# hank-kuo-cs/Volumetric-Primitives-Net

Hardware: AMD Instinct MI355X
Metric: render+Chamfer fwd+bwd images/sec (higher is better)
Workload: dtype f32; 1 GPU; C3: B=64/GPU (global 64), K=32 sphere primitives, 256x256 silhouette+depth, n=256 pts/prim (N=8192) vs M=2048 GT points, Chamfer+L1 fwd+bwd; global_batch=64, parallelism=dp1, collective=none, sampling=fresh Philox draws every step (device step counter, 28 steps drawn)

## Files before the change

### volumetric-primitives-net_amd/csrc/chamfer.hip

```cpp
#include "vpn_common.h"
#include "vpn_chamfer_feat.h"
#include "vpn_chamfer_loss.h"
#include "vpn_raster_common.h"
#include <stdlib.h>
#include <string.h>
#include <type_traits>

#pragma clang fp contract(off)

namespace vpn {

constexpr int CH_BLOCK = 256;
constexpr int CH_WTILE = 256;

typedef float f2 __attribute__((ext_vector_type(2)));

#ifdef CM_EXP_TRACE
__device__ unsigned long long g_ctrace[8192 * 8];
extern "C" int vpn_debug_scan_trace(void* dst, int nwg) {
    return (int)hipMemcpyFromSymbol(dst, HIP_SYMBOL(g_ctrace), (size_t)nwg * 8 * sizeof(unsigned long long), 0, hipMemcpyDeviceToDevice);
}
#endif
#ifdef VPN_CHAMFER_DEBUG
__device__ unsigned long long g_dbg[8];
// ... 776 lines not shown
    constexpr int FQ = THREADS >= 512 ? CM_FQ : 2;
    constexpr int UN = CM_FUN;
    __shared__ unsigned long long key[FQ];
    const int n4 = Ntp >> 2;
    const float4* f4 = reinterpret_cast<const float4*>(Fb);
    if (threadIdx.x < FQ) key[threadIdx.x] = ~0ull;
    for (int k0 = 0; k0 < count; k0 += FQ) {
        float mx[FQ], my[FQ], mz[FQ], thr[FQ];
#pragma unroll
        for (int c = 0; c < FQ; ++c) {
            const int k = min(k0 + c, count - 1);
            const float4 a = lqd[k];
            const float na = a.x * a.x + a.y * a.y + a.z * a.z;
            const float sab = sqrt_up(na) + snb;
            const float E = CM_EPS * (sab * sab) * (1.0f + 1.0e-6f);
            const float m2 = a.w * a.w;
            float th = (m2 * (1.0f + 1.0e-5f) - na) + (E + 4.0e-7f * (m2 + na));
            th = th == th ? th : __builtin_inff();
            th = k0 + c < count ? th : -__builtin_inff();
            auto uni = [](float v) { return __int_as_float(__builtin_amdgcn_readfirstlane(__float_as_int(v))); };
            mx[c] = uni(-2.0f * a.x); my[c] = uni(-2.0f * a.y); mz[c] = uni(-2.0f * a.z); thr[c] = uni(th);
        }
        __syncthreads();
        for (int base = threadIdx.x; base < n4; base += UN * THREADS) {
            float4 x[UN], y[UN], z[UN];
#pragma unroll
            for (int u = 0; u < UN; ++u) {
                const int g4 = min(base + u * THREADS, n4 - 1);
                x[u] = f4[g4]; y[u] = f4[n4 + g4]; z[u] = f4[2 * n4 + g4];
            }
#pragma unroll
            for (int u = 0; u < UN; ++u) {
                if (base + u * THREADS >= n4) break;
                const float xs[4] = {x[u].x, x[u].y, x[u].z, x[u].w}, ys[4] = {y[u].x, y[u].y, y[u].z, y[u].w};
                const float zs[4] = {z[u].x, z[u].y, z[u].z, z[u].w};
                float ws[4];
#pragma unroll
                for (int e = 0; e < 4; ++e)
                    ws[e] = __builtin_fmaf(zs[e], zs[e], __builtin_fmaf(ys[e], ys[e], xs[e] * xs[e]));
#pragma unroll
                for (int c = 0; c < FQ; ++c) {
                    float t[4];
#pragma unroll
                    for (int e = 0; e < 4; ++e)
                        t[e] = __builtin_fmaf(mx[c], xs[e], __builtin_fmaf(my[c], ys[e], __builtin_fmaf(mz[c], zs[e], ws[e])));
                    if (fminf(fminf(fminf(t[0], t[1]), t[2]), t[3]) <= thr[c]) {
#pragma unroll
                        for (int e = 0; e < 4; ++e) {
                            const int j = (base + u * THREADS) * 4 + e;
                            if (t[e] <= thr[c] && j < Nt) {
                                const float d = dist2_exact(-0.5f * mx[c], -0.5f * my[c], -0.5f * mz[c], xs[e], ys[e], zs[e]);
                                atomicMin(&key[c], ((unsigned long long)__float_as_uint(sqrtf(d)) << 32) | (unsigned)j);
                            }
                        }
                    }
                }
            }
        }
        __syncthreads();
        if (threadIdx.x < FQ) {
            const int k = k0 + threadIdx.x;
            const unsigned long long best = key[threadIdx.x];
            key[threadIdx.x] = ~0ull;
            if (k < count) {
                const int qc = min(max(lqi[k].x, 0), Nq - 1);
                const float df = best != ~0ull ? __uint_as_float((unsigned)(best >> 32)) : lqd[k].w;
                out_dist[qc] = df;
                out_idx[qc] = best != ~0ull ? (int)(unsigned)best : lqi[k].y;
                lqd[k].w = df;
            }
        }
    }
}

struct ScanJob {
    const float* qpts; const float* F; const unsigned short* H; const unsigned int* nmax;
    int Nq, Nt, Ntp, gx, G;
    float* out_dist; int32_t* out_idx;
    float* wgsum;
    const int32_t* qperm;
    const float* tboxes;
    int cand;
    const float* qboxes;
};

template <int PREC>
#ifndef CM_WAVES_PER_EU
#define CM_WAVES_PER_EU 6
#endif
__global__ __launch_bounds__(cm_block<PREC>(), PREC == 1 ? 5 : CM_WAVES_PER_EU) void chamfer_nn_mfma_kernel(
    const ScanJob j0, const ScanJob j1, int nsamples, const RasterOrderJob oj) {
    __shared__ __attribute__((aligned(16))) unsigned char tileH16[PREC == 2 ? 2 * CM_TILE16 * CM_ROWB : 16];
    if constexpr (PREC == 2) {
        if ((int)blockIdx.x < oj.B) {
            __builtin_amdgcn_s_setprio(3);
            raster_order_wg<cm_block<PREC>()>(oj, (int)blockIdx.x, tileH16);
            return;
        }
    }
    const int wg = (int)blockIdx.x - (PREC == 2 ? oj.B : 0);
#ifdef CM_EXP_TRACE
    const unsigned long long t_start = wall_clock64();
    unsigned long long t_pro = t_start;
#endif
    __shared__ int s_cnt;
    if (threadIdx.x == 0) s_cnt = 0;
    const bool other = wg >= j0.G;
    const float* __restrict__ qpts = other ? j1.qpts : j0.qpts;
    const float* __restrict__ F = other ? j1.F : j0.F;
    const unsigned short* __restrict__ H = other ? j1.H : j0.H;
    const unsigned int* __restrict__ nmax = other ? j1.nmax : j0.nmax;
    const int Nq = other ? j1.Nq : j0.Nq, Nt = other ? j1.Nt : j0.Nt, Ntp = other ? j1.Ntp : j0.Ntp;
    const int gx = other ? j1.gx : j0.gx, G = other ? j1.G : j0.G;
    float* __restrict__ out_dist = other ? j1.out_dist : j0.out_dist;
    int32_t* __restrict__ out_idx = other ? j1.out_idx : j0.out_idx;
    float* __restrict__ wgsum = other ? j1.wgsum : j0.wgsum;
    const int32_t* __restrict__ qperm = PREC == 2 ? (other ? j1.qperm : j0.qperm) : nullptr;
    const float* __restrict__ tboxes = PREC == 2 ? (other ? j1.tboxes : j0.tboxes) : nullptr;
    const int cand = PREC == 2 ? (other ? j1.cand : j0.cand) : 0;
    const float* __restrict__ qboxes = PREC == 2 ? (other ? j1.qboxes : j0.qboxes) : nullptr;
    constexpr int QPW = cm_block<PREC>() / 2;
    constexpr int LISTB = QPW * 24 > (PREC == 2 ? 3 * CCAND_CAP * 4 : 0) ? QPW * 24 : 3 * CCAND_CAP * 4;
    __shared__ __attribute__((aligned(16))) unsigned char s_list[LISTB];
    float4* const s_qd = reinterpret_cast<float4*>(s_list);
    int2* const s_qi = reinterpret_cast<int2*>(s_list + QPW * 16);
    float* const s_cpl = reinterpret_cast<float*>(s_list);
    __shared__ unsigned short s_cidx[PREC == 2 ? CCAND_CAP : 2];
    int ccount = 0, cpad = 0;
    int vid = wg - (other ? j0.G : 0);
    {
        const int per = G >> 3;
        if (vid < (per << 3)) vid = (vid & 7) * per + (vid >> 3);
    }
    const int b = vid / gx, bx = vid - b * gx;
    const int wave = threadIdx.x >> 6, lane = threadIdx.x & 63, jq = lane & 31, half = lane >> 5;
    const float* qb = qpts + (size_t)b * Nq * 3;
    const int qi = (bx * (cm_block<PREC>() / 64) + wave) * 32 + jq;
    const int qc = qperm ? min(max(qperm[(size_t)b * ((Nq + 63) & ~63) + min(qi, Nq - 1)], 0), Nq - 1) : min(qi, Nq - 1);
    const F3 a3 = ld3(qb + qc * 3);
    const float ax = a3.x, ay = a3.y, az = a3.z;
    const float bq0 = half ? -2.0f * ay : -2.0f * ax;
    const float bq1 = half ? 1.0f : -2.0f * az;

    float best = __builtin_inff(), second = __builtin_inff();
    int blk = 0;
#define CM_SEL(dst, cond_mask, a, b) asm volatile("v_cndmask_b32 %0, %1, %2, %3" : "=v"(dst) : "v"(b), "v"(a), "s"(cond_mask))
#define CM_UPDATE(m, tb0)                                                                      \
    {                                                                                          \
        const int t_ = (tb0);                                                                  \
        unsigned long long k1_;                                                                \
        asm volatile("v_cmp_lt_f32 %0, %1, %2" : "=s"(k1_) : "v"(m), "v"(best));               \
        second = __builtin_amdgcn_fmed3f(best, second, (m));                                   \
        CM_SEL(blk, k1_, t_, blk);                                           \
        asm volatile("v_min_f32 %0, %1, %2" : "=v"(best) : "v"(best), "v"(m));                 \
    }
#define CM_UPDATE_C(m, J)                                                                      \
    {                                                                                          \
        unsigned long long k1_;                                                                \
        asm volatile("v_cmp_lt_f32 %0, %1, %2" : "=s"(k1_) : "v"(m), "v"(best));               \
        second = __builtin_amdgcn_fmed3f(best, second, (m));                                   \
        asm volatile("v_cndmask_b32 %0, %1, " #J ", %2" : "=v"(blkc) : "v"(blkc), "s"(k1_));   \
        asm volatile("v_min_f32 %0, %1, %2" : "=v"(best) : "v"(best), "v"(m));                 \
    }
    const float* Fb = F + (size_t)b * 4 * Ntp;
    const f16v zero = {0.f, 0.f, 0.f, 0.f, 0.f, 0.f, 0.f, 0.f, 0.f, 0.f, 0.f, 0.f, 0.f, 0.f, 0.f, 0.f};
    if constexpr (PREC == 2) {
        unsigned char (*tileH)[CM_TILE16 * CM_ROWB] = reinterpret_cast<unsigned char (*)[CM_TILE16 * CM_ROWB]>(tileH16);
        const unsigned char* Hb = reinterpret_cast<const unsigned char*>(H) + (size_t)b * Ntp * CM_ROWB16;
        h8 bq;
        {
            _Float16 qx[2], qy[2], qz[2];
            split2_f16(-2.0f * CM_S16 * ax, qx); split2_f16(-2.0f * CM_S16 * ay, qy); split2_f16(-2.0f * CM_S16 * az, qz);
            auto slot = [&](int k) -> _Float16 {
                if (k < 9) {
                    const int c = k / 3, t = k % 3;
                    const _Float16 v0 = c == 0 ? qx[0] : (c == 1 ? qy[0] : qz[0]);
                    const _Float16 v1 = c == 0 ? qx[1] : (c == 1 ? qy[1] : qz[1]);
                    return t == 1 ? v1 : v0;
                }
                return k == 9 ? (_Float16)32768.0f : (k == 10 ? (_Float16)16.0f : (k == 11 ? (_Float16)1.0f : (_Float16)0.0f));
            };
#pragma unroll
            for (int e = 0; e < 8; ++e) bq[e] = half ? slot(8 + e) : slot(e);
        }
        constexpr int F4 = CM_TILE16 * CM_ROWB16 / 16 / CM_BLOCK16;
        static_assert(F4 == 2 || F4 == 1, "tile fetch is written for 1 or 2 float4 per lane");
        const float4* Hq = reinterpret_cast<const float4*>(Hb) + threadIdx.x;
        struct Pre { float4 a, b; };
        auto fetch = [&](int t0) -> Pre {
            const float4* p = Hq + t0 * (CM_ROWB16 / 16);
            if constexpr (F4 == 2) return Pre{p[0], p[CM_BLOCK16]};
            else return Pre{p[0], p[0]};
        };
        const int f0 = threadIdx.x, f1 = threadIdx.x + CM_BLOCK16;
        const int o0 = (f0 >> 1) * CM_ROWB + (f0 & 1) * 16, o1 = (f1 >> 1) * CM_ROWB + (f1 & 1) * 16;
        auto stash = [&](int buf, const Pre& v) {
            *reinterpret_cast<float4*>(&tileH[buf][o0]) = v.a;
            if constexpr (F4 == 2) *reinterpret_cast<float4*>(&tileH[buf][o1]) = v.b;
        };
        auto rd = [&](const unsigned char* T, int blkk) -> float4 {
            return *reinterpret_cast<const float4*>(T + blkk * 32 * CM_ROWB);
        };
        auto block = [&](const float4& o) {
            return __builtin_amdgcn_mfma_f32_32x32x16_f16(__builtin_bit_cast(h8, o), bq, zero, 0, 0, 0);
        };
        static_assert(CM_TILE16 == 256, "the tile loop below is unrolled for 8 blocks per tile");
#define CM_PRIO(p)
#define CM_PAIR(oa, ob, J)                                                                     \
    {                                                                                          \
        CM_PRIO(1)                                                                             \
        const f16v accA = block(oa), accB = block(ob);                                         \
        CM_PRIO(0)                                                                             \
        const float mAB = min32(accA, accB);                                                   \
        CM_UPDATE_C(mAB, J)                                                                    \
    }
        float skipc = __builtin_inff();
        const float* __restrict__ tbox = tboxes ? tboxes + (size_t)b * (Ntp >> 5) * CFEAT_BOXF : nullptr;
        if (tbox) {
            const float nb0 = __uint_as_float(wave_max_bits(lane < CFEAT_SLOTS ? nmax[b * CFEAT_SLOTS + lane] : 0u));
            const float na0 = ax * ax + ay * ay + az * az;
            const float r = sqrt_up(na0) + sqrt_up(nb0), r2 = r * r;
            const float E0 = CM_EPS_F16 * r2 * (1.0f + 1.0e-6f) + 5.9604644775390625e-08f * 1.7320509f * r;
            if (nb0 <= CM_DOMAIN16 && na0 <= CM_DOMAIN16) skipc = (na0 + E0) + (3.0e-5f * r2 + 1.0e-30f);
        }
#define CM_SCAN_TILE(T, t0, nblk)                                                              \
    {                                                                                          \
        const float before = best;                                                             \
        float4 a0 = rd(T, 0), a1 = rd(T, 1), b0 = rd(T, 2), b1 = rd(T, 3);                     \
        CM_PAIR(a0, a1, 0)                                                                     \
        if (nblk > 2) {                                                                        \
            a0 = rd(T, 4); a1 = rd(T, 5);                                                      \
            CM_PAIR(b0, b1, 1)                                                                 \
            if (nblk > 4) {                                                                    \
                b0 = rd(T, 6); b1 = rd(T, 7);                                                  \
                CM_PAIR(a0, a1, 2)                                                             \
                if (nblk > 6) CM_PAIR(b0, b1, 3)                                               \
            }                                                                                  \
        }                                                                                      \
        blk = best < before ? (t0) + (blkc << 6) : blk;    \
    }
#define CM_QUADS(oa, ob, J0, J1, J2, J3)                                                       \
    {                                                                                          \
        const f16v accA = block(oa), accB = block(ob);                                         \
        const float q0 = min8<0>(accA), q1 = min8<8>(accA), q2 = min8<0>(accB), q3 = min8<8>(accB); \
        CM_UPDATE_C(q0, J0)                                                                    \
        CM_UPDATE_C(q1, J1)                                                                    \
        CM_UPDATE_C(q2, J2)                                                                    \
        CM_UPDATE_C(q3, J3)                                                                    \
    }
#define CM_SCAN_TILE_Q(T, t0, nblk)                                                            \
    {                                                                                          \
        const float before = best;                                                             \
        float4 a0 = rd(T, 0), a1 = rd(T, 1), b0 = rd(T, 2), b1 = rd(T, 3);                     \
        CM_QUADS(a0, a1, 0, 1, 2, 3)                                                           \
        if (nblk > 2) {                                                                        \
            a0 = rd(T, 4); a1 = rd(T, 5);                                                      \
            CM_QUADS(b0, b1, 4, 5, 6, 7)                                                       \
            if (nblk > 4) {                                                                    \
                b0 = rd(T, 6); b1 = rd(T, 7);                                                  \
                CM_QUADS(a0, a1, 8, 9, 10, 11)                                                 \
                if (nblk > 6) CM_QUADS(b0, b1, 12, 13, 14, 15)                                 \
            }                                                                                  \
        }                                                                                      \
        blk = best < before ? (t0) + (blkc << 4) : blk;    \
    }
        int buf = 0, blkc = 0;
        if (cand) {
            __shared__ float s_cred[8][CM_WAVES16];
            __shared__ int s_cwn[2][CM_WAVES16];
            const float inf = __builtin_inff();
            auto uni = [](float v) { return __int_as_float(__builtin_amdgcn_readfirstlane(__float_as_int(v))); };
            float cc[3];
            bool boxed = false;
            if (qboxes && !qperm) {
                const float* qbox = qboxes + ((size_t)b * (((Nq + 63) & ~63) >> 5) + bx) * CFEAT_BOXF;
                const float4 bl = *reinterpret_cast<const float4*>(qbox);
                const float2 bh = *reinterpret_cast<const float2*>(qbox + 4);
                const float lo[3] = {bl.x, bl.y, bl.z}, hi[3] = {bl.w, bh.x, bh.y};
                boxed = true;
#pragma unroll
                for (int a = 0; a < 3; ++a) {
                    boxed = boxed && fabsf(lo[a]) < inf && fabsf(hi[a]) < inf;
                    cc[a] = uni((lo[a] + hi[a]) * 0.5f);
                }
            }
            if (!boxed) {
                {
                    const float l0 = feat_wave_minmax<false>(ax), l1 = feat_wave_minmax<false>(ay), l2 = feat_wave_minmax<false>(az);
                    const float h0 = feat_wave_minmax<true>(ax), h1 = feat_wave_minmax<true>(ay), h2 = feat_wave_minmax<true>(az);
                    if (lane == 0) {
                        s_cred[0][wave] = l0; s_cred[1][wave] = l1; s_cred[2][wave] = l2;
                        s_cred[3][wave] = h0; s_cred[4][wave] = h1; s_cred[5][wave] = h2;
                    }
                }
                __syncthreads();
#pragma unroll
                for (int a = 0; a < 3; ++a) {
                    float l = s_cred[a][0], h = s_cred[3 + a][0];
#pragma unroll
                    for (int w = 1; w < CM_WAVES16; ++w) { l = fminf(l, s_cred[a][w]); h = fmaxf(h, s_cred[3 + a][w]); }
                    cc[a] = uni((l + h) * 0.5f);
                }
            }
            const int n4 = Ntp >> 2;
            const float4* f4 = reinterpret_cast<const float4*>(Fb);
            {
                float r2 = dist2_exact(ax, ay, az, cc[0], cc[1], cc[2]);
                r2 = r2 == r2 ? r2 : inf;
                float dmin = inf;
                for (int g = threadIdx.x; g < n4; g += CM_BLOCK16) {
                    const float4 X = f4[g], Y = f4[n4 + g], Z = f4[2 * n4 + g];
                    const float xs[4] = {X.x, X.y, X.z, X.w}, ys[4] = {Y.x, Y.y, Y.z, Y.w}, zs[4] = {Z.x, Z.y, Z.z, Z.w};
#pragma unroll
                    for (int e = 0; e < 4; ++e) {
                        const float d = dist2_exact(xs[e], ys[e], zs[e], cc[0], cc[1], cc[2]);
                        dmin = 4 * g + e < Nt ? fminf(dmin, d) : dmin;
                    }
                }
                r2 = feat_wave_minmax<true>(r2); dmin = feat_wave_minmax<false>(dmin);
                if (lane == 0) { s_cred[6][wave] = r2; s_cred[7][wave] = dmin; }
            }
            __syncthreads();
            float thr;
            {
                float r2 = s_cred[6][0], dc2 = s_cred[7][0];
#pragma unroll
                for (int w = 1; w < CM_WAVES16; ++w) { r2 = fmaxf(r2, s_cred[6][w]); dc2 = fminf(dc2, s_cred[7][w]); }
                const float R = (2.0f * sqrt_up(r2) + sqrt_up(dc2)) * (1.0f + 1.0e-6f);
                thr = uni((R * R) * (1.0f + CCAND_EPS) + CCAND_FLOOR);
            }
            int total = CCAND_CAP + 1;
            if (thr < inf) {
                total = 0;
                int pass = 0;
                for (int g0 = 0; g0 < n4; g0 += CM_BLOCK16, pass ^= 1) {
                    const int g = g0 + (int)threadIdx.x, gl = min(g, n4 - 1);
                    const float4 X = f4[gl], Y = f4[n4 + gl], Z = f4[2 * n4 + gl];
                    const float xs[4] = {X.x, X.y, X.z, X.w}, ys[4] = {Y.x, Y.y, Y.z, Y.w}, zs[4] = {Z.x, Z.y, Z.z, Z.w};
                    bool keep[4];
                    int before = 0, wtot = 0;
#pragma unroll
                    for (int e = 0; e < 4; ++e) {
                        const float d = dist2_exact(xs[e], ys[e], zs[e], cc[0], cc[1], cc[2]);
                        keep[e] = !(d > thr) && 4 * g + e < Nt;
                        const unsigned long long m = __ballot(keep[e]);
                        before += __popcll(m & ((1ull << lane) - 1ull));
                        wtot += __popcll(m);
                    }
                    if (lane == 0) s_cwn[pass][wave] = wtot;
                    __syncthreads();
                    int pos = total + before, all = 0;
#pragma unroll
                    for (int w = 0; w < CM_WAVES16; ++w) { const int c = s_cwn[pass][w]; pos += w < wave ? c : 0; all += c; }
#pragma unroll
                    for (int e = 0; e < 4; ++e) {
                        if (keep[e]) {
                            if (pos < CCAND_CAP) {
                                const int j = 4 * g + e;
                                s_cidx[pos] = (unsigned short)j;
                                s_cpl[pos] = xs[e]; s_cpl[CCAND_CAP + pos] = ys[e]; s_cpl[2 * CCAND_CAP + pos] = zs[e];
                                const uint4* hr = reinterpret_cast<const uint4*>(Hb + (size_t)j * CM_ROWB16);
                                const uint4 r0 = hr[0], r1 = hr[1];
                                *reinterpret_cast<uint4*>(&tileH16[pos * CM_ROWB]) = r0;
                                *reinterpret_cast<uint4*>(&tileH16[pos * CM_ROWB + 16]) = r1;
                            }
                            ++pos;
                        }
                    }
                    total = __builtin_amdgcn_readfirstlane(total + all);
                    if (total > CCAND_CAP) break;
                }
            }
            if (total >= 1 && total <= CCAND_CAP) {
                ccount = total; cpad = (total + 63) & ~63;
                const int p = total + (int)threadIdx.x;
                if (p < cpad) {
                    const Row16 pad = sentinel_row16();
                    s_cidx[p] = 0;
                    s_cpl[p] = 0.0f; s_cpl[CCAND_CAP + p] = 0.0f; s_cpl[2 * CCAND_CAP + p] = 0.0f;
                    *reinterpret_cast<uint4*>(&tileH16[p * CM_ROWB]) = pad.lo;
                    *reinterpret_cast<uint4*>(&tileH16[p * CM_ROWB + 16]) = pad.hi;
                }
            }
            __syncthreads();
        }
#ifdef CM_EXP_TRACE
        t_pro = wall_clock64();
#endif
        if (cpad) {
            for (int t0 = 0; t0 < cpad; t0 += CM_TILE16) {
                const int nblk = min(CM_TILE16, cpad - t0) >> 5;
                const unsigned char* T = &tileH16[(t0 + jq) * CM_ROWB + half * 16];
                CM_SCAN_TILE_Q(T, t0, nblk)
            }
        } else {
        Pre pre = fetch(0);
        stash(0, pre);
        __syncthreads();
        for (int t0 = 0; t0 < Ntp; t0 += CM_TILE16, buf ^= 1) {
            const bool more = t0 + CM_TILE16 < Ntp;
            if (more) pre = fetch(t0 + CM_TILE16);
            bool scan = true;
            if (tbox) {
                const float4 bl = *reinterpret_cast<const float4*>(tbox + (t0 >> 8) * CFEAT_BOXF);
                const float2 bh = *reinterpret_cast<const float2*>(tbox + (t0 >> 8) * CFEAT_BOXF + 4);
                const float dx = fmaxf(fmaxf(bl.x - ax, ax - bl.w), 0.0f);
                const float dy = fmaxf(fmaxf(bl.y - ay, ay - bh.x), 0.0f);
                const float dz = fmaxf(fmaxf(bl.z - az, az - bh.y), 0.0f);
                const float L = ((dx * dx + dy * dy) + dz * dz) * (1.0f - 1.0e-6f);
                scan = __ballot(!(L > __builtin_fmaf(best, CM_INV_S16SQ, skipc))) != 0ull;
#ifdef VPN_CHAMFER_DEBUG
                if (!scan && lane == 0) atomicAdd(&g_dbg[3], 1ull);
#endif
            }
            if (scan) {
            const int nblk = min(CM_TILE16, Ntp - t0) >> 5;
            const unsigned char* T = &tileH[buf][jq * CM_ROWB + half * 16];
            CM_SCAN_TILE(T, t0, nblk)
            }
            if (more) stash(buf ^ 1, pre);
            __syncthreads();
        }
        }
#undef CM_SCAN_TILE_Q
#undef CM_QUADS
#undef CM_SCAN_TILE
#undef CM_PAIR
    } else     if constexpr (PREC == 1) {
        __shared__ __attribute__((aligned(16))) unsigned char tileH[2][CM_TILE16 * CM_ROWB];
        const unsigned char* Hb = reinterpret_cast<const unsigned char*>(H) + (size_t)b * Ntp * CM_ROWB;
        bf8 bqA;
        bs4 bqB;
        {
            unsigned short qx[3], qy[3], qz[3];
            split3_bf16(-2.0f * ax, qx); split3_bf16(-2.0f * ay, qy); split3_bf16(-2.0f * az, qz);
            auto slot = [&](int k) -> unsigned short {
                const int c = k / 6, t = k % 6;
                const int pi = (t == 1 || t == 5) ? 1 : (t == 3 ? 2 : 0);
                if (k < 18) {
                    const unsigned short v0 = c == 0 ? qx[0] : (c == 1 ? qy[0] : qz[0]);
                    const unsigned short v1 = c == 0 ? qx[1] : (c == 1 ? qy[1] : qz[1]);
                    const unsigned short v2 = c == 0 ? qx[2] : (c == 1 ? qy[2] : qz[2]);
                    return pi == 0 ? v0 : (pi == 1 ? v1 : v2);
                }
                return k < 21 ? (unsigned short)0x3F80 : (unsigned short)0;
            };
            us8 ua;
            us4 ub;
#pragma unroll
            for (int e = 0; e < 8; ++e) ua[e] = half ? slot(8 + e) : slot(e);
#pragma unroll
            for (int e = 0; e < 4; ++e) ub[e] = half ? slot(20 + e) : slot(16 + e);
            bqA = __builtin_bit_cast(bf8, ua); bqB = __builtin_bit_cast(bs4, ub);
        }
        constexpr int F4 = CM_TILE16 * CM_ROWB / 16 / CM_BLOCK;
        static_assert(F4 == 3, "tile fetch is written for 3 float4 per lane");
        const float4* Hq = reinterpret_cast<const float4*>(Hb) + threadIdx.x;
        struct Pre { float4 a, b, c; };
        auto fetch = [&](int t0) -> Pre {
            const float4* p = Hq + t0 * (CM_ROWB / 16);
            return Pre{p[0], p[CM_BLOCK], p[2 * CM_BLOCK]};
        };
        auto stash = [&](int buf, const Pre& v) {
            float4* q = reinterpret_cast<float4*>(&tileH[buf][0]) + threadIdx.x;
            q[0] = v.a; q[CM_BLOCK] = v.b; q[2 * CM_BLOCK] = v.c;
        };
        struct Ops { float4 lo; float2 hi; };
        auto rd = [&](const unsigned char* T, int blkk) -> Ops {
            const unsigned char* p = T + blkk * 32 * CM_ROWB;
            return Ops{*reinterpret_cast<const float4*>(p), *reinterpret_cast<const float2*>(p + 32 - 8 * half)};
        };
        auto block = [&](const Ops& o) {
            f16v acc = __builtin_amdgcn_mfma_f32_32x32x16_bf16(__builtin_bit_cast(bf8, o.lo), bqA, zero, 0, 0, 0);
            acc = __builtin_amdgcn_mfma_f32_32x32x8bf16_1k(__builtin_bit_cast(bs4, o.hi), bqB, acc, 0, 0, 0);
            return acc;
        };
        static_assert(CM_TILE16 == 256, "the tile loop below is unrolled for 8 blocks per tile");
// ... 462 lines not shown
#pragma unroll
            for (int r = 0; r < CPR_RING; ++r) {
                if (i + r < cnt) {
                    process(ring[r], kk[r]);
                    if (i + r + CPR_RING < cnt) { kk[r] = base + (int)__builtin_ctzll(m); m &= m - 1; ring[r] = ld(kk[r]); }
                }
            }
        }
    }
    int K;
    float Bv, V2;
    {
        const float ob = __shfl_xor(best, 32, 64), os = __shfl_xor(second, 32, 64);
        const int ok = __shfl_xor(blk, 32, 64);
        Bv = fminf(best, ob);
        K = (ob < best || (ob == best && ok < blk)) ? ok : blk;
        V2 = fminf(K == blk ? second : best, K == ok ? os : ob);
    }
    float d2[16];
    int og[16];
    float m2 = __builtin_inff();
    {
        const int base = K + half * 16;
        const float4* px4 = reinterpret_cast<const float4*>(Fb + base);
        const float4* py4 = reinterpret_cast<const float4*>(Fb + (size_t)Ntp + base);
        const float4* pz4 = reinterpret_cast<const float4*>(Fb + 2 * (size_t)Ntp + base);
        const int4* pm4 = reinterpret_cast<const int4*>(permt + (size_t)b * Ntp + base);
        float4 X[4], Y[4], Z[4];
        int4 P[4];
#pragma unroll
        for (int v = 0; v < 4; ++v) { X[v] = px4[v]; Y[v] = py4[v]; Z[v] = pz4[v]; P[v] = pm4[v]; }
#pragma unroll
        for (int v = 0; v < 4; ++v) {
            const float xs[4] = {X[v].x, X[v].y, X[v].z, X[v].w}, ys[4] = {Y[v].x, Y[v].y, Y[v].z, Y[v].w};
            const float zs[4] = {Z[v].x, Z[v].y, Z[v].z, Z[v].w};
            const int ps[4] = {P[v].x, P[v].y, P[v].z, P[v].w};
#pragma unroll
            for (int w = 0; w < 4; ++w) {
                const int e = v * 4 + w;
                og[e] = ps[w];
                d2[e] = dist2_exact(ax, ay, az, xs[w], ys[w], zs[w]) + ((base + e < Nt) ? 0.0f : __builtin_inff());
                m2 = fminf(m2, d2[e]);
            }
        }
    }
    m2 = fminf(m2, __shfl_xor(m2, 32, 64));
    const float band = E + 4.0e-6f * (m2 + na);
    const float s = sqrtf(m2);
    const float band_near = near_error(CM_EPS_BF16, 0.0f, na, sqrt_up(na), s * (1.0f + 1.0e-7f), E) + 4.0e-6f * (m2 + na);
    const bool ambiguous = !(V2 > (m2 - na) + band_near) || !(m2 - na <= Bv + band);
    const float lim = m2 * (1.0f + 1.0e-6f);
    int idx = 0x7fffffff;
    bool near_tie = false;
#pragma unroll
    for (int e = 0; e < 16; ++e) {
        if (d2[e] == m2) idx = min(idx, og[e]);
        near_tie |= (d2[e] != m2) && (d2[e] <= lim);
    }
    if (__ballot(near_tie)) {
#pragma unroll
        for (int e = 0; e < 16; ++e)
            if (d2[e] <= lim && sqrtf(d2[e]) == s) idx = min(idx, og[e]);
    }
    idx = min(idx, __shfl_xor(idx, 32, 64));
    if (half == 0 && pos < Nq) {
        const int oq = permq[(size_t)b * Nqp + pos];
        out_dist[(size_t)b * Nq + oq] = s;
        out_idx[(size_t)b * Nq + oq] = idx;
        if (ambiguous)
            reinterpret_cast<int4*>(undecided + pad4(nsamples))[(size_t)b * Nq + atomicAdd(undecided + b, 1)] =
                make_int4(oq, __float_as_int(ax), __float_as_int(ay), __float_as_int(az));
    }
}

static int chamfer_cand() {
    static int on = -1;
    if (on < 0) {
        const char* e = getenv("VPN_CHAMFER_CAND");
        on = !(e && e[0] == '0') ? 1 : 0;
    }
    return on;
}

static inline int pad32(int n) { return (n + 63) & ~63; }
static inline int wgsum_per_sample(int Nq) { return (Nq + 127) / 128; }
static inline size_t mfma_ws_floats(int B, int Nt, int Nq) {
    return (size_t)B * (4 + CM_ROWW) * pad32(Nt) + (size_t)CM_TILE16 * CM_ROWW + (size_t)B * CFEAT_SLOTS + (size_t)pad4(B) + 4 * (size_t)B * Nq
           + (size_t)B * pad32(Nt) + (size_t)B * (pad32(Nt) / 32) * CS_BOXF
           + (size_t)pad4(B * wgsum_per_sample(Nq));
}

static inline int feat_split(int Ntp) { const int y = (Ntp + CFEAT_WGPTS - 1) / CFEAT_WGPTS; return y > CFEAT_SLOTS ? CFEAT_SLOTS : y; }
struct MfmaWs { float* F; unsigned short* H; unsigned int* nmax; int* undecided; int32_t* perm; float* boxes; float* wgsum; int Ntp; };

static MfmaWs mfma_carve(float* F, int B, int Nt, int Nq) {
    MfmaWs w;
    w.Ntp = pad32(Nt);
    w.F = F;
    w.H = reinterpret_cast<unsigned short*>(F + (size_t)B * 4 * w.Ntp);
    w.nmax = reinterpret_cast<unsigned int*>(F + (size_t)B * (4 + CM_ROWW) * w.Ntp + (size_t)CM_TILE16 * CM_ROWW);
    w.undecided = reinterpret_cast<int*>(w.nmax + (size_t)B * CFEAT_SLOTS);
    w.perm = reinterpret_cast<int32_t*>(w.undecided + pad4(B) + 4 * (size_t)B * Nq);
    w.boxes = reinterpret_cast<float*>(w.perm + (size_t)B * w.Ntp);
    w.wgsum = w.boxes + (size_t)B * (w.Ntp / 32) * CS_BOXF;
    return w;
}

static int mfma_both(const float* p1, const float* p2, int B, int N, int M, float* ws, float* d1, int32_t* i1, float* d2,
                     int32_t* i2, int prec, hipStream_t s, bool features_ready = false,
                     const RasterOrderJob* rider = nullptr) {
    const bool fp32_filter = prec == 0;
    const MfmaWs w2 = mfma_carve(ws, B, M, N);
    const MfmaWs w1 = mfma_carve(ws + mfma_ws_floats(B, M, N), B, N, M);
    auto split = [](int Ntp) { return feat_split(Ntp); };
    const bool skip = prec == 2 && N >= CSKIP_MIN_TARGETS;
    auto cand = [&](int Nq, int Nt, const float* boxes) {
        return chamfer_cand() && prec == 2 && !boxes && Nq >= CSKIP_MIN_TARGETS && Nt <= CCAND_MAX_TARGETS ? 1 : 0;
    };
    const FeatJob f2{p2, M, w2.Ntp, split(w2.Ntp), w2.F, w2.nmax, fp32_filter ? nullptr : w2.H, prec == 2, nullptr,
                     skip ? w2.perm : nullptr};
    const FeatJob f1{p1, N, w1.Ntp, split(w1.Ntp), w1.F, w1.nmax, fp32_filter ? nullptr : w1.H, prec == 2,
                     skip ? w1.boxes : nullptr, nullptr};
    hipError_t e = hipSuccess;
    if (!features_ready) {
        const int ord = skip ? (B + 7) & ~7 : 0;
        VPN_LAUNCH(chamfer_feat_kernel, dim3(ord + B * (f2.ysplit + f1.ysplit)), dim3(CFEAT_THREADS), 0, s, f2, f1, B, ord);
        e = hipGetLastError();
        if (e != hipSuccess) return (int)e;
    }
    {
        const int qpw = prec == 2 ? 32 * CM_WAVES16 : 128;
        const int gx1 = (N + qpw - 1) / qpw, gx2 = (M + qpw - 1) / qpw;
        const ScanJob s1{p1, w2.F, w2.H, w2.nmax, N, M, w2.Ntp, gx1, gx1 * B, d1, i1, w2.wgsum, nullptr, nullptr,
                         cand(N, M, nullptr), f1.tboxes};
        const ScanJob s2{p2, w1.F, w1.H, w1.nmax, M, N, w1.Ntp, gx2, gx2 * B, d2, i2, w1.wgsum,
                         f2.perm, f1.tboxes, cand(M, N, f1.tboxes), nullptr};
        const bool long_first = (long long)N > (long long)M;
        const ScanJob& ja = long_first ? s2 : s1;
        const ScanJob& jb = long_first ? s1 : s2;
        const RasterOrderJob none{};
        if (prec == 0)
            VPN_LAUNCH(chamfer_nn_mfma_kernel<0>, dim3(ja.G + jb.G), dim3(CM_BLOCK), 0, s, ja, jb, B, none);
        else if (prec == 1)
            VPN_LAUNCH(chamfer_nn_mfma_kernel<1>, dim3(ja.G + jb.G), dim3(CM_BLOCK), 0, s, ja, jb, B, none);
        else
            VPN_LAUNCH(chamfer_nn_mfma_kernel<2>, dim3(ja.G + jb.G + (rider ? rider->B : 0)), dim3(CM_BLOCK16), 0, s, ja, jb, B,
                       rider ? *rider : none);
        e = hipGetLastError();
        if (e != hipSuccess) return (int)e;
    }
    return 0;
}

static int chamfer_mode();
int chamfer_feat_jobs(void* workspace, size_t workspace_bytes, int B, int N, int M, const float* p1, const float* p2,
                      FeatJob* job1, FeatJob* job2) {
    if (!workspace || B <= 0 || N <= 0 || M <= 0 || ((uintptr_t)workspace & 15) != 0) return VPN_E_BADARG;
    if (workspace_bytes < vpn_chamfer_workspace(B, N, M)) return VPN_E_BADARG;
    const int forced = chamfer_mode();
    if (!(forced == 6 || (forced == 0 && (long)N * M >= 512L * 512L))) return VPN_E_BADARG;
    float* ws = (float*)workspace;
    const MfmaWs w2 = mfma_carve(ws, B, M, N);
    const MfmaWs w1 = mfma_carve(ws + mfma_ws_floats(B, M, N), B, N, M);
    const bool skip = N >= CSKIP_MIN_TARGETS;
    *job2 = FeatJob{p2, M, w2.Ntp, feat_split(w2.Ntp), w2.F, w2.nmax, w2.H, 1, nullptr, skip ? w2.perm : nullptr};
    *job1 = FeatJob{p1, N, w1.Ntp, feat_split(w1.Ntp), w1.F, w1.nmax, w1.H, 1, skip ? w1.boxes : nullptr, nullptr};
    return 0;
}

int chamfer_wgsums(const void* workspace, size_t workspace_bytes, int B, int N, int M, const float** sums1, int* g1,
                   const float** sums2, int* g2) {
    if (!workspace || B <= 0 || N <= 0 || M <= 0 || ((uintptr_t)workspace & 15) != 0) return VPN_E_BADARG;
    if (workspace_bytes < vpn_chamfer_workspace(B, N, M)) return VPN_E_BADARG;
    const int forced = chamfer_mode();
    if (!(forced == 6 || (forced == 0 && (long)N * M >= 512L * 512L))) return VPN_E_BADARG;
    float* ws = (float*)const_cast<void*>(workspace);
    const MfmaWs w2 = mfma_carve(ws, B, M, N);
    const MfmaWs w1 = mfma_carve(ws + mfma_ws_floats(B, M, N), B, N, M);
    const int qpw = 32 * CM_WAVES16;
    *sums1 = w2.wgsum; *g1 = (N + qpw - 1) / qpw;
    *sums2 = w1.wgsum; *g2 = (M + qpw - 1) / qpw;
    return 0;
}

struct CloudWs { float* sorted; int32_t* perm; float* boxes; int C; };

static inline int chunks_of(int N) { return (N + CP_CHUNK - 1) / CP_CHUNK; }
static inline size_t cloud_ws_floats(int B, int N) { return (size_t)B * ((size_t)N * 4 + (size_t)chunks_of(N) * 6); }

static CloudWs carve(float*& cur, int B, int N) {
    CloudWs w;
    w.C = chunks_of(N);
    w.sorted = cur; cur += (size_t)B * N * 3;
    w.perm = reinterpret_cast<int32_t*>(cur); cur += (size_t)B * N;
    w.boxes = cur; cur += (size_t)B * w.C * 6;
    return w;
}

static int pruned_nn(const CloudWs& q, const CloudWs& t, int B, int Nq, int Nt, float* d, int32_t* idx, hipStream_t s) {
    dim3 grid((Nq + 63) / 64, B);
    VPN_LAUNCH(chamfer_nn_pruned_kernel<1>, grid, dim3(64), 0, s, q.sorted, q.perm, t.sorted, t.perm, t.boxes,
                       Nq, Nt, t.C, d, idx);
    hipError_t e = hipGetLastError();
    return e == hipSuccess ? 0 : (int)e;
}

static int mfma_sorted_both(const float* p1, const float* p2, int B, int N, int M, float* ws, float* d1, int32_t* i1,
                            float* d2, int32_t* i2, hipStream_t s) {
    const MfmaWs w2 = mfma_carve(ws, B, M, N);
    const MfmaWs w1 = mfma_carve(ws + mfma_ws_floats(B, M, N), B, N, M);
    const SortJob s2{p2, M, w2.Ntp, w2.F, w2.nmax, w2.H, w2.undecided, w2.perm, w2.boxes};
    const SortJob s1{p1, N, w1.Ntp, w1.F, w1.nmax, w1.H, w1.undecided, w1.perm, w1.boxes};
    VPN_LAUNCH(chamfer_sortfeat_kernel, dim3(2 * B), dim3(CS_THREADS), 0, s, s2, s1, B);
    hipError_t e = hipGetLastError();
    if (e != hipSuccess) return (int)e;
    for (int dir = 0; dir < 2; ++dir) {
        const MfmaWs& wq = dir ? w2 : w1;
        const MfmaWs& wt = dir ? w1 : w2;
        const int Nq = dir ? M : N, Nt = dir ? N : M;
// ... 172 lines not shown
```

Before: 439,500 images/s.

## Order target tiles by box distance and cull per group in GT→pred Chamfer scan

Adds a new scan path for the second Chamfer direction (GT queries against predicted points with tile boxes). It sorts the target tiles by the distance from their bounding boxes to the workgroup's query centroid. Tiles are then visited in groups of four, and a tile is skipped when no lane's current best distance could beat its box bound. Visiting near tiles first should tighten the best distance early and prune more far tiles. The cost is an extra wave reduction, a rank sort and per-group barriers plus shared-memory need-bit voting, which may outweigh the savings when little gets culled.

```diff
diff --git a/volumetric-primitives-net_amd/csrc/chamfer.hip b/volumetric-primitives-net_amd/csrc/chamfer.hip
--- a/volumetric-primitives-net_amd/csrc/chamfer.hip
+++ b/volumetric-primitives-net_amd/csrc/chamfer.hip
@@ -882,6 +882,7 @@
     const float* tboxes;
     int cand;
     const float* qboxes;
+    int dorder;
 };
 
 template <int PREC>
@@ -919,6 +920,7 @@
     const float* __restrict__ tboxes = PREC == 2 ? (other ? j1.tboxes : j0.tboxes) : nullptr;
     const int cand = PREC == 2 ? (other ? j1.cand : j0.cand) : 0;
     const float* __restrict__ qboxes = PREC == 2 ? (other ? j1.qboxes : j0.qboxes) : nullptr;
+    const int dorder = PREC == 2 ? (other ? j1.dorder : j0.dorder) : 0;
     constexpr int QPW = cm_block<PREC>() / 2;
     constexpr int LISTB = QPW * 24 > (PREC == 2 ? 3 * CCAND_CAP * 4 : 0) ? QPW * 24 : 3 * CCAND_CAP * 4;
     __shared__ __attribute__((aligned(16))) unsigned char s_list[LISTB];
@@ -1065,9 +1067,9 @@
         blk = best < before ? (t0) + (blkc << 4) : blk;    \
     }
         int buf = 0, blkc = 0;
+        __shared__ float s_cred[8][CM_WAVES16];
+        __shared__ int s_cwn[2][CM_WAVES16];
         if (cand) {
-            __shared__ float s_cred[8][CM_WAVES16];
-            __shared__ int s_cwn[2][CM_WAVES16];
             const float inf = __builtin_inff();
             auto uni = [](float v) { return __int_as_float(__builtin_amdgcn_readfirstlane(__float_as_int(v))); };
             float cc[3];
@@ -1193,6 +1195,130 @@
                 const unsigned char* T = &tileH16[(t0 + jq) * CM_ROWB + half * 16];
                 CM_SCAN_TILE_Q(T, t0, nblk)
             }
+        } else if (tbox && dorder && ((Ntp + CM_TILE16 - 1) >> 8) <= LISTB / (CFEAT_BOXF * 4)) {
+#ifndef CD2_GROUP
+#define CD2_GROUP 4
+#endif
+            constexpr int CD2_G = CD2_GROUP;
+            static_assert(CM_WAVES16 == 8 && CD2_G <= 8, "one byte of need bits per wave, read as two 32-bit words");
+            unsigned char* const s_ord = reinterpret_cast<unsigned char*>(&s_cred[6][0]);
+            unsigned char* const s_need = reinterpret_cast<unsigned char*>(&s_cwn[0][0]);
+            const float inf = __builtin_inff();
+            const int nt = (Ntp + CM_TILE16 - 1) >> 8;
+            const bool ordered = (dorder & 1) && nt <= 64;
+            float* const s_box = reinterpret_cast<float*>(s_list);
+            static_assert(2 * (LISTB / (CFEAT_BOXF * 4)) <= CM_BLOCK16, "one float4 of the boxes per lane");
+            if ((int)threadIdx.x < 2 * nt)
+                reinterpret_cast<float4*>(s_box)[threadIdx.x] = reinterpret_cast<const float4*>(tbox)[threadIdx.x];
+            if (!ordered) __syncthreads();
+            if (ordered) {
+                {
+                    const float l0 = feat_wave_minmax<false>(ax), l1 = feat_wave_minmax<false>(ay), l2 = feat_wave_minmax<false>(az);
+                    const float h0 = feat_wave_minmax<true>(ax), h1 = feat_wave_minmax<true>(ay), h2 = feat_wave_minmax<true>(az);
+                    if (lane == 0) {
+                        s_cred[0][wave] = l0; s_cred[1][wave] = l1; s_cred[2][wave] = l2;
+                        s_cred[3][wave] = h0; s_cred[4][wave] = h1; s_cred[5][wave] = h2;
+                    }
+                }
+                __syncthreads();
+                if (wave == 0) {
+                    float c[3];
+                    bool fin = true;
+#pragma unroll
+                    for (int a = 0; a < 3; ++a) {
+                        float l = s_cred[a][0], h = s_cred[3 + a][0];
+#pragma unroll
+                        for (int w = 1; w < CM_WAVES16; ++w) { l = fminf(l, s_cred[a][w]); h = fmaxf(h, s_cred[3 + a][w]); }
+                        c[a] = (l + h) * 0.5f;
+                        fin = fin && fabsf(c[a]) < inf;
+                    }
+                    const float* bp = s_box + min(lane, nt - 1) * CFEAT_BOXF;
+                    const float4 bl = *reinterpret_cast<const float4*>(bp);
+                    const float2 bh = *reinterpret_cast<const float2*>(bp + 4);
+                    const float dx = fmaxf(fmaxf(bl.x - c[0], c[0] - bl.w), 0.0f);
+                    const float dy = fmaxf(fmaxf(bl.y - c[1], c[1] - bh.x), 0.0f);
+                    const float dz = fmaxf(fmaxf(bl.z - c[2], c[2] - bh.y), 0.0f);
+                    float key = (dx * dx + dy * dy) + dz * dz;
+                    key = key == key ? key : inf;
+                    int rank = 0;
+                    for (int j = 0; j < nt; ++j) {
+                        const float kj = __int_as_float(__builtin_amdgcn_readlane(__float_as_int(key), j));
+                        rank += (kj < key || (kj == key && j < lane)) ? 1 : 0;
+                    }
+                    if (lane < nt) s_ord[fin ? rank : lane] = (unsigned char)lane;
+                }
+                __syncthreads();
+            }
+#ifdef CM_EXP_TRACE
+            t_pro = wall_clock64();
+#endif
+            auto tile_at = [&](int p) -> int {
+                return ordered ? __builtin_amdgcn_readfirstlane((int)s_ord[p]) : p;
+            };
+            auto wanted = [&](int tile) -> bool {
+                const float4 bl = *reinterpret_cast<const float4*>(s_box + tile * CFEAT_BOXF);
+                const float2 bh = *reinterpret_cast<const float2*>(s_box + tile * CFEAT_BOXF + 4);
+                const float dx = fmaxf(fmaxf(bl.x - ax, ax - bl.w), 0.0f);
+                const float dy = fmaxf(fmaxf(bl.y - ay, ay - bh.x), 0.0f);
+                const float dz = fmaxf(fmaxf(bl.z - az, az - bh.y), 0.0f);
+                const float L = ((dx * dx + dy * dy) + dz * dz) * (1.0f - 1.0e-6f);
+                return __ballot(!(L > __builtin_fmaf(best, CM_INV_S16SQ, skipc))) != 0ull;
+            };
+            int p0 = 0, par = 0;
+            unsigned mine = (1u << min(nt, CD2_G)) - 1u;
+            unsigned need = mine & ~1u;
+            bool dirty = false;
+            int pos = 0, t0 = tile_at(0) << 8;
+            Pre pre = fetch(t0);
+            stash(0, pre);
+            __syncthreads();
+            for (;;) {
+                bool scan = (mine >> (pos - p0)) & 1u;
+                const bool again = dirty;
+                while (need == 0u && p0 + CD2_G < nt) {
+                    p0 += CD2_G; par ^= 1;
+                    mine = 0u;
+                    if (dorder & 2) {
+#pragma unroll
+                        for (int g = 0; g < CD2_G; ++g)
+                            if (p0 + g < nt && wanted(tile_at(p0 + g))) mine |= 1u << g;
+                    } else {
+                        mine = (1u << min(nt - p0, CD2_G)) - 1u;
+                    }
+                    dirty = !(dorder & 2);
+                    if (__builtin_amdgcn_mbcnt_hi(~0u, __builtin_amdgcn_mbcnt_lo(~0u, 0u)) == 0u)
+                        s_need[par * 8 + __builtin_amdgcn_readfirstlane(wave)] = (unsigned char)mine;
+                    __syncthreads();
+                    const unsigned* nw = reinterpret_cast<const unsigned*>(s_need + par * 8);
+                    unsigned x = nw[0] | nw[1];
+                    x |= x >> 16; x |= x >> 8;
+                    need = (unsigned)__builtin_amdgcn_readfirstlane((int)(x & 0xffu));
+                }
+                const bool more = need != 0u;
+                int posn = pos, t0n = t0;
+                if (more) {
+                    posn = p0 + __builtin_ctz(need);
+                    need &= need - 1u;
+                    t0n = tile_at(posn) << 8;
+                    pre = fetch(t0n);
+                }
+                if (scan && again) scan = wanted(t0 >> 8);
+#ifdef VPN_CHAMFER_DEBUG
+                if (!scan && lane == 0) atomicAdd(&g_dbg[3], 1ull);
+                if (threadIdx.x == 0) atomicAdd(&g_dbg[0], 1ull);
+#endif
+                if (scan) {
+                    const int nblk = min(CM_TILE16, Ntp - t0) >> 5;
+                    const unsigned char* T = &tileH[buf][jq * CM_ROWB + half * 16];
+                    CM_SCAN_TILE(T, t0, nblk)
+                    dirty = true;
+                }
+                if (!more) break;
+                stash(buf ^ 1, pre);
+                __syncthreads();
+                buf ^= 1; pos = posn; t0 = t0n;
+            }
+            __syncthreads();
         } else {
         Pre pre = fetch(0);
         stash(0, pre);
@@ -1821,6 +1947,15 @@
     return on;
 }
 
+static int chamfer_d2order() {
+    static int v = -1;
+    if (v < 0) {
+        const char* e = getenv("VPN_CHAMFER_D2ORDER");
+        v = e && e[0] >= '0' && e[0] <= '2' ? e[0] - '0' : 3;
+    }
+    return v;
+}
+
 static inline int pad32(int n) { return (n + 63) & ~63; }
 static inline int wgsum_per_sample(int Nq) { return (Nq + 127) / 128; }
 static inline size_t mfma_ws_floats(int B, int Nt, int Nq) {
@@ -1871,9 +2006,9 @@
         const int qpw = prec == 2 ? 32 * CM_WAVES16 : 128;
         const int gx1 = (N + qpw - 1) / qpw, gx2 = (M + qpw - 1) / qpw;
         const ScanJob s1{p1, w2.F, w2.H, w2.nmax, N, M, w2.Ntp, gx1, gx1 * B, d1, i1, w2.wgsum, nullptr, nullptr,
-                         cand(N, M, nullptr), f1.tboxes};
+                         cand(N, M, nullptr), f1.tboxes, 0};
         const ScanJob s2{p2, w1.F, w1.H, w1.nmax, M, N, w1.Ntp, gx2, gx2 * B, d2, i2, w1.wgsum,
-                         f2.perm, f1.tboxes, cand(M, N, f1.tboxes), nullptr};
+                         f2.perm, f1.tboxes, cand(M, N, f1.tboxes), nullptr, chamfer_d2order()};
         const bool long_first = (long long)N > (long long)M;
         const ScanJob& ja = long_first ? s2 : s1;
         const ScanJob& jb = long_first ? s1 : s2;
```

Result: faster. 447,100 images/s (median of 6 runs) (+1.7%).

## Add per-wave box-culled tile walk for GT-to-prediction Chamfer scan

Applied to the files above, without the earlier changes.

Adds a new scan path for the boxed target job, enabled by default through an environment switch. Each wave walks the target tiles on its own, skipping tiles whose bounding box cannot beat the current best distance. It loads rows straight from global memory through buffer loads, with a rotating register pipeline that prefetches the next wanted tile. This removes the shared-memory staging and the workgroup-wide barriers of the cooperative tile loop. In exchange, waves diverge, loads go uncoalesced from L2, and there is more inline-asm complexity.

```diff
diff --git a/volumetric-primitives-net_amd/csrc/chamfer.hip b/volumetric-primitives-net_amd/csrc/chamfer.hip
--- a/volumetric-primitives-net_amd/csrc/chamfer.hip
+++ b/volumetric-primitives-net_amd/csrc/chamfer.hip
@@ -882,6 +882,7 @@
     const float* tboxes;
     int cand;
     const float* qboxes;
+    int walk;
 };
 
 template <int PREC>
@@ -919,6 +920,7 @@
     const float* __restrict__ tboxes = PREC == 2 ? (other ? j1.tboxes : j0.tboxes) : nullptr;
     const int cand = PREC == 2 ? (other ? j1.cand : j0.cand) : 0;
     const float* __restrict__ qboxes = PREC == 2 ? (other ? j1.qboxes : j0.qboxes) : nullptr;
+    const int walk = PREC == 2 ? (other ? j1.walk : j0.walk) : 0;
     constexpr int QPW = cm_block<PREC>() / 2;
     constexpr int LISTB = QPW * 24 > (PREC == 2 ? 3 * CCAND_CAP * 4 : 0) ? QPW * 24 : 3 * CCAND_CAP * 4;
     __shared__ __attribute__((aligned(16))) unsigned char s_list[LISTB];
@@ -1193,6 +1195,100 @@
                 const unsigned char* T = &tileH16[(t0 + jq) * CM_ROWB + half * 16];
                 CM_SCAN_TILE_Q(T, t0, nblk)
             }
+        } else if (tbox && walk) {
+            __syncthreads();
+            const unsigned loff = (unsigned)(jq * CM_ROWB16 + half * 16);
+            const __amdgpu_buffer_rsrc_t rows =
+                __builtin_amdgcn_make_buffer_rsrc(const_cast<unsigned char*>(Hb), 0, Ntp * CM_ROWB16, 0x00020000);
+            auto ldb = [&](int t0, int k) -> float4 {
+                return __builtin_bit_cast(float4, __builtin_amdgcn_raw_buffer_load_b128(
+                    rows, loff, (t0 + 32 * k) * CM_ROWB16, 0));
+            };
+            typedef float cbox4 __attribute__((ext_vector_type(4)));
+            typedef float cbox2 __attribute__((ext_vector_type(2)));
+            const __attribute__((address_space(4))) float* cbox = (const __attribute__((address_space(4))) float*)(uintptr_t)tbox;
+            auto wanted = [&](int t0) -> bool {
+                const cbox4 bl = *(const __attribute__((address_space(4))) cbox4*)(cbox + (t0 >> 8) * CFEAT_BOXF);
+                const cbox2 bh = *(const __attribute__((address_space(4))) cbox2*)(cbox + (t0 >> 8) * CFEAT_BOXF + 4);
+                const float dx = fmaxf(fmaxf(bl.x - ax, ax - bl.w), 0.0f);
+                const float dy = fmaxf(fmaxf(bl.y - ay, ay - bh.x), 0.0f);
+                const float dz = fmaxf(fmaxf(bl.z - az, az - bh.y), 0.0f);
+                const float L = ((dx * dx + dy * dy) + dz * dz) * (1.0f - 1.0e-6f);
+                return __ballot(!(L > __builtin_fmaf(best, CM_INV_S16SQ, skipc))) != 0ull;
+            };
+            auto next = [&](int t0) -> int {
+                while (t0 < Ntp && !wanted(t0)) t0 += CM_TILE16;
+                return t0;
+            };
+#ifdef VPN_CHAMFER_DEBUG
+            int nscan = 0;
+#define CM_WALK_COUNT ++nscan;
+#else
+#define CM_WALK_COUNT
+#endif
+#define CM_PAIR_W(oa, ob, J)                                                                   \
+    {                                                                                          \
+        const f16v accA = block(oa), accB = block(ob);                                         \
+        const float mAB = min32(accA, accB);                                                   \
+        unsigned long long k1_;                                                                \
+        asm volatile("v_cmp_lt_f32 %0, %1, %2" : "=s"(k1_) : "v"(mAB), "v"(best));             \
+        asm volatile("v_med3_f32 %0, %1, %0, %2" : "+v"(second) : "v"(best), "v"(mAB));        \
+        asm volatile("v_cndmask_b32 %0, %1, " #J ", %2" : "=v"(blkc) : "v"(blkc), "s"(k1_));   \
+        asm volatile("v_min_f32 %0, %1, %2" : "=v"(best) : "v"(best), "v"(mAB));               \
+    }
+#define CM_WALK_TILE(A, B, C, D, E, F)                                                         \
+    {                                                                                          \
+        if (!wanted(tc)) {                        \
+            tc = next(tc + CM_TILE16);                                                         \
+            if (tc >= Nfull) break;                                                            \
+            A = ldb(tc, 0); B = ldb(tc, 1); C = ldb(tc, 2); D = ldb(tc, 3);                    \
+        }                                                                                      \
+        CM_WALK_COUNT                                                                          \
+        blkc = -1;                                \
+        E = ldb(tc, 4); F = ldb(tc, 5);                                                        \
+        CM_PAIR_W(A, B, 0)                                                                     \
+        A = ldb(tc, 6); B = ldb(tc, 7);                                                        \
+        CM_PAIR_W(C, D, 1)                                                                     \
+        const int tn = next(tc + CM_TILE16);      \
+        const int tl = tn < Nfull ? tn : tc;                                                   \
+        C = ldb(tl, 0); D = ldb(tl, 1);                                                        \
+        CM_PAIR_W(E, F, 2)                                                                     \
+        E = ldb(tl, 2); F = ldb(tl, 3);                                                        \
+        CM_PAIR_W(A, B, 3)                                                                     \
+        blk = blkc >= 0 ? tc + (blkc << 6) : blk;        \
+        tc = tn;                                                                               \
+        if (tc >= Nfull) break;                                                                \
+    }
+            const int Nfull = Ntp & ~(CM_TILE16 - 1);
+            int tc = next(0);
+            if (tc < Nfull) {
+                float4 r0 = ldb(tc, 0), r1 = ldb(tc, 1), r2 = ldb(tc, 2), r3 = ldb(tc, 3);
+                float4 r4 = make_float4(0.f, 0.f, 0.f, 0.f), r5 = r4;
+                for (;;) {
+                    CM_WALK_TILE(r0, r1, r2, r3, r4, r5)
+                    CM_WALK_TILE(r2, r3, r4, r5, r0, r1)
+                    CM_WALK_TILE(r4, r5, r0, r1, r2, r3)
+                }
+            }
+            if (tc < Ntp && wanted(tc)) {
+                const int nblk = (Ntp - tc) >> 5;
+                CM_WALK_COUNT
+                const float before = best;
+                float4 a0 = ldb(tc, 0), a1 = ldb(tc, 1), b0 = ldb(tc, 2), b1 = ldb(tc, 3);
+                CM_PAIR(a0, a1, 0)
+                if (nblk > 2) {
+                    a0 = ldb(tc, 4); a1 = ldb(tc, 5);
+                    CM_PAIR(b0, b1, 1)
+                    if (nblk > 4) CM_PAIR(a0, a1, 2)
+                }
+                blk = best < before ? tc + (blkc << 6) : blk;
+            }
+#ifdef VPN_CHAMFER_DEBUG
+            if (lane == 0) atomicAdd(&g_dbg[3], (unsigned long long)((Ntp + CM_TILE16 - 1) / CM_TILE16 - nscan));
+#endif
+#undef CM_WALK_TILE
+#undef CM_PAIR_W
+#undef CM_WALK_COUNT
         } else {
         Pre pre = fetch(0);
         stash(0, pre);
@@ -1821,6 +1917,15 @@
     return on;
 }
 
+static int chamfer_wavewalk() {
+    static int on = -1;
+    if (on < 0) {
+        const char* e = getenv("VPN_CHAMFER_WAVEWALK");
+        on = !(e && e[0] == '0') ? 1 : 0;
+    }
+    return on;
+}
+
 static inline int pad32(int n) { return (n + 63) & ~63; }
 static inline int wgsum_per_sample(int Nq) { return (Nq + 127) / 128; }
 static inline size_t mfma_ws_floats(int B, int Nt, int Nq) {
@@ -1871,9 +1976,9 @@
         const int qpw = prec == 2 ? 32 * CM_WAVES16 : 128;
         const int gx1 = (N + qpw - 1) / qpw, gx2 = (M + qpw - 1) / qpw;
         const ScanJob s1{p1, w2.F, w2.H, w2.nmax, N, M, w2.Ntp, gx1, gx1 * B, d1, i1, w2.wgsum, nullptr, nullptr,
-                         cand(N, M, nullptr), f1.tboxes};
+                         cand(N, M, nullptr), f1.tboxes, 0};
         const ScanJob s2{p2, w1.F, w1.H, w1.nmax, M, N, w1.Ntp, gx2, gx2 * B, d2, i2, w1.wgsum,
-                         f2.perm, f1.tboxes, cand(M, N, f1.tboxes), nullptr};
+                         f2.perm, f1.tboxes, cand(M, N, f1.tboxes), nullptr, chamfer_wavewalk()};
         const bool long_first = (long long)N > (long long)M;
         const ScanJob& ja = long_first ? s2 : s1;
         const ScanJob& jb = long_first ? s1 : s2;
```

New measurement: 438,300 images/s before, 459,100 images/s after (median of 6 runs). +4.8%, better.
